# mozack/vdjer

Hardware: AMD Instinct MI355X
Metric: M paired-reads/sec (k-mer build + contig score), IgH 50bp PE (higher is better)
Workload: dtype u8/u64 (2-bit packed bases, integer counts)

## Files before the change

### vdjer_amd/csrc/vdjx_kmer.hip

```cpp
#include "vdjx_common.h"
#include "vdjx_scan.h"
#include "vdjx_part.h"

#include <algorithm>
#include <numeric>
#include <type_traits>
#include <string.h>
#include <stdlib.h>

#define HIST_THREADS 512
#define HIST_BLOCKS 512u
#define LOCAL_SLOTS 2048u
#define K3_SUB_TUPLES g_sub_tuples
__device__ u32 g_sub_tuples = 262144u;
#define NONE32 0xFFFFFFFFu
#define INST_MASK 0x7FFFFFFFu

struct RecView {
	u64 bhi, blo, nm, lq;
};

__device__ inline RecView load_rec(const u64* __restrict__ bases, const u64* __restrict__ nmask,
                                   const u64* __restrict__ lowq, size_t r) {
	RecView v;
// ... 164 lines not shown
			u32 at = incl - c;
			for (u32 gg = g; gg; gg &= gg - 1) wl[at++] = (uint16_t) ((lane << (LONG ? 8 : 6)) | (u32) (ob + __builtin_ctz(gg)));
			vdjx_wave_lds_fence();
			if (dbg == 2) { sink += wl[lane]; vdjx_wave_lds_fence(); continue; }
			for (u32 i = lane; i < total; i += 64) {
				const u32 e = wl[i];
				u64 khi, klo;
				if (LONG) vdjx_kmer_at_words(wrow + (e >> 8) * GL_ROW_LONG, k, (int) (e & 255u), khi, klo);
				else if (SYM) (void) sym_canonical(wb[e >> 6], rl, k, (int) (e & 63u), khi, klo);
				else {
					const ulonglong2 bb = wb[e >> 6];
					vdjx_kmer_at_lane(bb.x, bb.y, rl, k, (int) (e & 63u), khi, klo);
				}
				if (dbg == 3) { sink += (u32) (vdjx_bucket_mix(klo, khi) >> (64 - nb_bits)); continue; }
				atomicAdd(&hist[(u32) (vdjx_bucket_mix(klo, khi) >> (64 - nb_bits))], 1u);
			}
			vdjx_wave_lds_fence();
		}
	}
	__syncthreads();
	if (dbg) { if (sink == 0x12345u) bucket_cnt[0] = sink; return; }
	for (u32 i = threadIdx.x; i < NB; i += HIST_THREADS) if (hist[i]) atomicAdd(&bucket_cnt[i], hist[i]);
}

template <typename TUP> struct TupBucket {
	u32 shift, mask;
	__device__ inline u32 operator()(const TUP& t) const { return (u32) (vdjx_bucket_mix(t.lo, t.hi()) >> shift) & mask; }
};

#define PARTR_STAGE_BYTES 98304u
template <typename TUP, bool LONG, bool SYM = false>
__global__ __launch_bounds__(PART_THREADS) void k_part_records_g(const u64* __restrict__ bases, const u64* __restrict__ nmask,
                                                                 const u64* __restrict__ lowq, size_t R, u64 rec_base, int rl, int k,
                                                                 u32 shift, u32 nbk, size_t rpb, u32 rr0, u32* __restrict__ gcur,
                                                                 TUP* __restrict__ out) {
	extern __shared__ __attribute__((aligned(16))) uint8_t smem[];
	TUP* stage = (TUP*) smem;
	u32* desc = (u32*) (smem + PARTR_STAGE_BYTES);
	__shared__ part_round pr;
	__shared__ u32 s_n;
	constexpr u32 ROUND = PARTR_STAGE_BYTES / sizeof(TUP);
	constexpr int OB = LONG ? 8 : 6;
	const int P = rl - k + 1;
	const u32 rr_min = ROUND / (u32) P;
	u32 rr = rr0 > rr_min ? rr0 : rr_min;
	const u32 mask = nbk - 1;
	const u32 lane = threadIdx.x & 63u, wave = threadIdx.x >> 6;
	static_assert(!(LONG && SYM), "SYM is the short-read form");
	uint8_t* wv = smem + wave * (LONG ? GL_WAVE_BYTES_LONG : GL_WAVE_BYTES);
	ulonglong2* wb = (ulonglong2*) wv;
	u64* wrow = (u64*) wv;
	uint16_t* wl = (uint16_t*) (wv + (LONG ? 64u * GL_ROW_LONG * 8u : 1024u));
	const size_t r0 = (size_t) blockIdx.x * rpb;
	const size_t r1 = r0 + rpb < R ? r0 + rpb : R;
	size_t rs = r0;
	while (rs < r1) {
		const size_t re = rs + rr < r1 ? rs + rr : r1;
		if (threadIdx.x == 0) s_n = 0;
		pr.begin(nbk);
		for (size_t rb = rs; rb < re; rb += PART_THREADS) {
			const size_t r = rb + threadIdx.x;
			u64 G = 0;
			vdjx_mask3 bad{~0ull, ~0ull, ~0ull};
			if (r < re) {
				if (LONG) { bad = load_gate3(lowq, r); stage_row_long(wrow + lane * GL_ROW_LONG, bases, r); }
				else {
					const GateView v = load_gate(bases, lowq, SYM ? 2 * r : r);
// ... 7 lines not shown
				const u32 g = LONG ? vdjx_clean16(bad, ob, k, P) : (u32) (G >> ob) & 0xFFFFu;
				const u32 c = (u32) __popc(g);
				const u32 incl = (u32) vdjx_wave_scan_add((int) c);
				const u32 total = (u32) __builtin_amdgcn_readlane((int) incl, 63);
				if (!total) continue;
				u32 at = incl - c;
				for (u32 gg = g; gg; gg &= gg - 1) wl[at++] = (uint16_t) ((lane << OB) | (u32) (ob + __builtin_ctz(gg)));
				vdjx_wave_lds_fence();
				u32 dbase = 0;
				if (lane == 0) dbase = atomicAdd(&s_n, total);
				dbase = (u32) __builtin_amdgcn_readlane((int) dbase, 0);
				for (u32 i = lane; i < total; i += 64) {
					const u32 e = wl[i];
					u64 khi, klo;
					if (LONG) vdjx_kmer_at_words(wrow + (e >> 8) * GL_ROW_LONG, k, (int) (e & 255u), khi, klo);
					else if (SYM) (void) sym_canonical(wb[e >> 6], rl, k, (int) (e & 63u), khi, klo);
					else {
						const ulonglong2 bb = wb[e >> 6];
						vdjx_kmer_at_lane(bb.x, bb.y, rl, k, (int) (e & 63u), khi, klo);
					}
					const u32 b = (u32) (vdjx_bucket_mix(klo, khi) >> shift) & mask;
					pr.count(b);
					if (dbase + i < ROUND) desc[dbase + i] = ((loc0 + (e >> OB)) << (OB + 10)) | ((e & ((1u << OB) - 1u)) << 10) | b;
				}
				vdjx_wave_lds_fence();
			}
		}
		__syncthreads();
		if (s_n > ROUND) {
			rr = rr / 2 > rr_min ? rr / 2 : rr_min;
			__syncthreads();
			continue;
		}
		const u32 n = pr.reserve(nbk, gcur);
		for (u32 i = threadIdx.x; i < n; i += PART_THREADS) {
			const u32 d = desc[i];
			const size_t r = rs + (d >> (OB + 10));
			const u32 o = (d >> 10) & ((1u << OB) - 1u);
			u64 khi, klo;
			u64 inst = ((rec_base + (u64) r) << OB) | (u64) o;
			if (LONG) vdjx_kmer_at_words(bases + r * VDJX_LONG_W, k, (int) o, khi, klo);
			else if (SYM) {
				const bool flip = sym_canonical(((const ulonglong2*) bases)[2 * r], rl, k, (int) o, khi, klo);
				inst = flip ? ((rec_base + 2 * (u64) r + 1) << OB) | (u64) (rl - k - (int) o) : ((rec_base + 2 * (u64) r) << OB) | (u64) o;
			} else {
				const ulonglong2 bb = ((const ulonglong2*) bases)[r];
				vdjx_kmer_at_lane(bb.x, bb.y, rl, k, (int) o, khi, klo);
			}
			TUP::store(&stage[pr.slot(d & 1023u)], TUP::make(klo, khi, inst));
		}
		__syncthreads();
		pr.flush(stage, n, out, TupBucket<TUP>{shift, mask});
		rs = re;
	}
}

template <typename TUP>
__global__ __launch_bounds__(512) void k_seg_hist_g(const TUP* __restrict__ in, const u32* __restrict__ seg_start, u32 seg_shift, u32 slices,
                                                    u32 shift, u32 sub_bits, u32* __restrict__ fine_cnt) {
	__shared__ u32 h[PART_MAXB];
	const u32 nbk = 1u << sub_bits;
	for (u32 i = threadIdx.x; i < nbk; i += 512) h[i] = 0;
	__syncthreads();
	size_t t0, t1;
	const u32 seg = part_slice(seg_start, seg_shift, slices, t0, t1);
	for (size_t t = t0 + threadIdx.x; t < t1; t += 512) {
		const TUP x = TUP::load(&in[t]);
// ... 1607 lines not shown
	explicit PersistAlloc(vdjx_ctx* ctx) : c(ctx) {}
	template <typename T> hipError_t alloc(T** out, size_t n) {
		*out = (T*) c->shard_arena.alloc((n ? n : 1) * sizeof(T));
		return *out ? hipSuccess : hipErrorOutOfMemory;
	}
	vdjx_arena::mark_t mark() const { return c->shard_arena.mark(); }
	void release_to(vdjx_arena::mark_t m) { c->shard_arena.release_to(m); }
};

struct PoolView { const u64* bases; const u64* nmask; vdjx_qrows quals; int rl; int ob; };

template <typename TUP> struct GTuples {
	TUP* t = nullptr;
	u32* bucket_start = nullptr;
	u32 NB = 0, N = 0;
};

struct SurvivorsG {
	u64 *lo = nullptr, *hi = nullptr, *gfirst = nullptr, *ufirst = nullptr;
	u32 *gcnt = nullptr, *ucnt = nullptr;
	u32 n = 0, n_real = 0;
	u64 ndist = 0;
};

inline u32 ceil_log2_u64(u64 x) { u32 b = 0; while ((1ull << b) < x) b++; return b; }

static bool sync_debug() { static const bool on = vdjx_env_set("VDJX_SYNC_DEBUG"); return on; }
static void dbg_sync(vdjx_ctx* c, const char* what) {
	if (!sync_debug()) return;
	const hipError_t e = hipStreamSynchronize(c->stream);
	fprintf(stderr, "[vdjx] %s: %s\n", what, hipGetErrorString(e));
}

struct GatedHist { u32 HB = 0, NBH = 0, N = 0; u32* hstart = nullptr; bool sym = false; };
static bool build_sym(const vdjx_pool* pool, int k) {
	return pool->sym && pool->W == 2 && (k & 1) && pool->n_records % 2 == 0;
}
static bool sym_walk_wanted() { static const bool on = !vdjx_env_set("VDJX_NO_SYM_WALK"); return on; }
static size_t gated_bucket_default() { static const size_t v = (size_t) vdjx_env_num("VDJX_GATED_BUCKET", 3072, 1, 1ll << 32); return v; }
template <typename A>
int stage_gated_hist(vdjx_ctx* c, A& db, const vdjx_pool* pool, int k, size_t per_bucket, u64 geometry_instances, GatedHist* gh, bool sym = false) {
	hipStream_t st = c->stream;
	const size_t R = sym ? pool->n_records / 2 : pool->n_records;
	const int P = pool->rl - k + 1;
	const u64 NI = geometry_instances ? geometry_instances : (u64) R * (u64) P;
	const size_t per = per_bucket ? per_bucket : gated_bucket_default();
	const u32 hb_max = pool->W > 2 ? 14u : 15u;
	u32 HB = ceil_log2_u64((NI + per - 1) / per);
	HB = std::max(8u, std::min(hb_max, HB));
	const u32 NBH = 1u << HB;
#ifdef VDJX_ABLATE
	static const u32 hist_dbg = (u32) vdjx_env_num("VDJX_HIST_DBG", 0, 0, 4);
#else
	constexpr u32 hist_dbg = 0;
#endif
	u32 nblk = (u32) std::min<size_t>(HIST_BLOCKS, (R + 4095) / 4096);
	if (nblk == 0) nblk = 1;
	size_t rpb = (R + nblk - 1) / nblk;
	u32 *hcnt, *hstart;
	HIP_TRY(db.alloc(&hcnt, NBH));
	HIP_TRY(db.alloc(&hstart, NBH + 1));
	HIP_TRY(hipMemsetAsync(hcnt, 0, (size_t) NBH * 4, st));
	const bool lng = pool->W > 2;
	const size_t lds_hist = (size_t) NBH * 4 + (HIST_THREADS / 64) * (lng ? GL_WAVE_BYTES_LONG : GL_WAVE_BYTES);
	HIP_TRY(hipFuncSetAttribute((const void*) k_gated_hist<false>, hipFuncAttributeMaxDynamicSharedMemorySize, (int) lds_hist));
	HIP_TRY(hipFuncSetAttribute((const void*) k_gated_hist<true>, hipFuncAttributeMaxDynamicSharedMemorySize, (int) lds_hist));
	HIP_TRY(hipFuncSetAttribute((const void*) k_gated_hist<false, true>, hipFuncAttributeMaxDynamicSharedMemorySize, (int) lds_hist));
	{
		vdjx_prof_scope ps(c, "k_gated_hist");
		if (lng) hipLaunchKernelGGL(k_gated_hist<true>, dim3(nblk), dim3(HIST_THREADS), lds_hist, st, pool->d_bases, pool->d_nmask, pool->d_lowq, R, pool->rl, k, HB, rpb, hcnt, hist_dbg);
		else if (sym) hipLaunchKernelGGL((k_gated_hist<false, true>), dim3(nblk), dim3(HIST_THREADS), lds_hist, st, pool->d_bases, pool->d_nmask, pool->d_lowq, R, pool->rl, k, HB, rpb, hcnt, hist_dbg);
		else hipLaunchKernelGGL(k_gated_hist<false>, dim3(nblk), dim3(HIST_THREADS), lds_hist, st, pool->d_bases, pool->d_nmask, pool->d_lowq, R, pool->rl, k, HB, rpb, hcnt, hist_dbg);
	}
	dbg_sync(c, "k_gated_hist");
	vdjx_scan_one(st, hcnt, NBH, hstart);
	HIP_TRY(hipMemcpyAsync(c->h_pin, hstart + NBH, 4, hipMemcpyDeviceToHost, st));
	HIP_TRY(hipStreamSynchronize(st));
	HIP_TRY(hipGetLastError());
#ifdef VDJX_ABLATE
	if (hist_dbg) return VDJX_ESTATE;
#endif
	const u32 N = *(const u32*) c->h_pin;
	c->stats["gated_instances"] = sym ? 2ull * N : N;
	gh->HB = HB; gh->NBH = NBH; gh->N = N; gh->hstart = hstart; gh->sym = sym;
	return VDJX_OK;
}

template <typename TUP, typename A>
int stage_gated_cut(vdjx_ctx* c, A& db, const vdjx_pool* pool, u64 rec_base, int k, size_t per_bucket, u64 geometry_instances, const GatedHist& gh, GTuples<TUP>* out) {
	hipStream_t st = c->stream;
	const bool sym = gh.sym;
	const size_t R = sym ? pool->n_records / 2 : pool->n_records;
	const int P = pool->rl - k + 1;
	const size_t per = per_bucket ? per_bucket : gated_bucket_default();
	const u32 hb_max = pool->W > 2 ? 14u : 15u;
	const bool lng = pool->W > 2;
	const u32 HB = gh.HB, NBH = gh.NBH, N = gh.N;
	u32* hstart = gh.hstart;
	size_t rpb;
	out->N = N;
	const u64 Ng = geometry_instances ? geometry_instances : (u64) N;
	static const size_t refine = (size_t) vdjx_env_num("VDJX_REFINE_TUPLES", 4096, 1, 1ll << 32);
	u32 T = 8;
	while (T < HB && ((u64) per << T) < Ng) T++;
	u32 extra = 0;
	const size_t refine_at = per_bucket ? std::max<size_t>(per_bucket, refine / 2) : refine;
	if (T == HB && HB == hb_max && Ng / NBH > refine_at) {
		extra = 1;
		while (extra < 5 && (Ng >> extra) / NBH > refine_at) extra++;
	}
	const u32 Tt = T + extra;
	const u32 NBt = 1u << Tt;
	HIP_TRY(db.alloc(&out->t, (size_t) N + 1));
	constexpr u32 stage_tuples = PARTR_STAGE_BYTES / (u32) sizeof(TUP);
	constexpr u32 lds_partr = PARTR_STAGE_BYTES + stage_tuples * 4;
	u32 cbits = Tt, fbits = 0;
	if (Tt > 10) { cbits = extra ? Tt - 10 : 8; fbits = Tt - cbits; }
	const u32 NBc = 1u << cbits;
	u32 nblk2 = (u32) std::min<size_t>(1024, (R + 2047) / 2048);
	if (nblk2 == 0) nblk2 = 1;
	rpb = (R + nblk2 - 1) / nblk2;
	u32* gcur;
	HIP_TRY(db.alloc(&gcur, NBc));
	TUP* l1 = out->t;
	if (fbits) HIP_TRY(db.alloc(&l1, (size_t) N + 1));
	{
		vdjx_prof_scope ps(c, "k_part_records");
		const u64 NIl = (u64) R * (u64) P;
		u64 rr = N ? (u64) stage_tuples * 3 / 4 * NIl / ((u64) N * (u64) P) : 1u << 16;
		rr = std::max<u64>(PART_THREADS, std::min<u64>(rr / PART_THREADS * PART_THREADS, lng ? 1u << 14 : 1u << 16));
		auto* part_records = lng ? k_part_records_g<TUP, true> : sym ? k_part_records_g<TUP, false, true> : k_part_records_g<TUP, false>;
		HIP_TRY(part_launch(st, part_records, nblk2, lds_partr, hstart, NBc, HB - cbits, gcur, l1, pool->d_bases, pool->d_nmask, pool->d_lowq, R, rec_base,
		                    pool->rl, k, 64 - cbits, NBc, rpb, (u32) rr));
	}
	dbg_sync(c, "k_part_records");
	u32* tstart;
	HIP_TRY(db.alloc(&tstart, NBt + 1));
	out->NB = NBt;
	out->bucket_start = tstart;
	constexpr u32 slices = PART_SLICES;
	if (extra) {
		u32* fine_cnt;
		HIP_TRY(db.alloc(&fine_cnt, NBt));
		HIP_TRY(hipMemsetAsync(fine_cnt, 0, (size_t) NBt * 4, st));
		vdjx_prof_scope ps(c, "k_seg_hist");
		hipLaunchKernelGGL(k_seg_hist_g<TUP>, dim3(NBc * slices), dim3(512), 0, st, l1, hstart, HB - cbits, slices, 64 - Tt, fbits, fine_cnt);
		vdjx_scan_one(st, fine_cnt, NBt, tstart);
	} else {
		hipLaunchKernelGGL(k_pick_u32, dim3((NBt + 1 + 255) / 256), dim3(256), 0, st, hstart, 1u << (HB - Tt), NBt + 1, tstart);
	}
	if (fbits) {
		u32* gcur2;
		HIP_TRY(db.alloc(&gcur2, NBt));
		vdjx_prof_scope ps(c, "k_part_tuples");
		HIP_TRY(part_launch(st, k_part<TUP, TupBucket<TUP>, part_segs>, NBc * slices, PART_LDS_BYTES, tstart, NBt, 0u, gcur2, out->t,
		                    l1, part_segs{hstart, HB - cbits, slices, fbits}, TupBucket<TUP>{64 - Tt, (1u << fbits) - 1u}));
	}
	return VDJX_OK;
}

template <typename TUP, typename A>
int stage_gated_partition(vdjx_ctx* c, A& db, const vdjx_pool* pool, u64 rec_base, int k, size_t per_bucket, u64 geometry_instances, GTuples<TUP>* out, bool sym = false) {
	GatedHist gh;
	int rc = stage_gated_hist(c, db, pool, k, per_bucket, geometry_instances, &gh, sym);
	if (rc) return rc;
	return stage_gated_cut<TUP>(c, db, pool, rec_base, k, per_bucket, geometry_instances, gh, out);
}

static int set_sub_tuples(vdjx_ctx* c) {
	static const u32 sub = (u32) vdjx_env_num("VDJX_SUB_TUPLES", 262144, 1, 0xFFFFFFFFll);
	if (c->sub_tuples_set != sub) {
		HIP_TRY(hipMemcpyToSymbolAsync(HIP_SYMBOL(g_sub_tuples), &sub, 4, 0, hipMemcpyHostToDevice, c->stream));
		c->sub_tuples_set = sub;
	}
	return VDJX_OK;
}
template <typename TUP, typename A>
int bucket_order(vdjx_ctx* c, A& db, const GTuples<TUP>& t, u32** order) {
	*order = nullptr;
	if (t.NB < 1024) return VDJX_OK;
	HIP_TRY(db.alloc(order, t.NB));
	hipLaunchKernelGGL(k_bucket_order, dim3(1), dim3(1024), 0, c->stream, t.bucket_start, t.NB, *order);
	return VDJX_OK;
}

template <typename TUP, typename A>
int stage_gated_reduce(vdjx_ctx* c, A& db, const GTuples<TUP>& t, const PoolView& pv, u64 rec_base, int k, int mf, int mq, SurvivorsG* sv, bool sym = false) {
	hipStream_t st = c->stream;
	int rc = set_sub_tuples(c);
// ... 150 lines not shown
		u32 x = f.mul;
		for (int i = 0; i < 5; i++) x *= 2u - f.mul * x;
		f.inv = x & f.bmask;
		f.ns = ns;
	}
	const u32 nsp = (f.bmask + 1u) << 4;
	static const bool force_wide = vdjx_env_num("VDJX_RC_WIDE", 0, 0, 1) != 0;
	static const u32 cap_shift = (u32) vdjx_env_num("VDJX_RC_MAX_SHIFT", 12, 8, 12);
	const bool narrow = R < (1ull << (32 - pool->ob)) && !force_wide;
	static const u32 max_ranges = (u32) vdjx_env_num("VDJX_RC_MAX_RANGES", PART_MAXB, 2, PART_MAXB);
	const u32 max_shift = std::max(8u, std::min(narrow ? 11u : 10u, cap_shift));
	u32 range_shift = 8;
	while (range_shift < max_shift && (nsp >> range_shift) > max_ranges) range_shift++;
	const u32 n_ranges = std::max(1u, nsp >> range_shift);
	u32 l2bits = 0;
	while (((n_ranges + (1u << l2bits) - 1) >> l2bits) > max_ranges) l2bits++;
	if (l2bits) l2bits = std::min(10u, std::max(l2bits, (ceil_log2_u64(n_ranges) + 1u) / 2u));
	const u32 n_coarse = (n_ranges + (1u << l2bits) - 1) >> l2bits;
	const u32 n_ranges_p = n_coarse << l2bits;
	constexpr size_t walk_blocks = 7168;
	const size_t Rw = sym_walk ? R / 2 : R;
	u32 nblk = (u32) std::min<size_t>(walk_blocks, (Rw + WALK_THREADS * 8 - 1) / (WALK_THREADS * 8));
	constexpr u32 walk_resident = 1536;
	if (nblk > walk_resident && nblk < walk_blocks) nblk = nblk / walk_resident * walk_resident;
	if (nblk < walk_resident) nblk = (u32) std::min<size_t>(walk_resident, (Rw + WALK_THREADS - 1) / WALK_THREADS);
	if (nblk == 0) nblk = 1;
	const size_t nwaves = (size_t) nblk * (WALK_THREADS / 64);
	const size_t NI = R * (size_t) P;
	u32 blk_items = 4096;
	while (blk_items > 256 && nwaves * blk_items > NI / 2 + 65536) blk_items >>= 1;
	const u64 raw_cap = (u64) NI + (u64) NI / (blk_items / 64) + nwaves * (u64) blk_items + blk_items;
	u64 *raw, *items;
	unsigned long long *g_cursor, *n_inst;
	u32 *range_cnt, *range_start, *g_err, *gcur;
	const vdjx_arena::mark_t tmp_mark = db.mark();
	HIP_TRY(db.alloc(&raw, (size_t) raw_cap));
	HIP_TRY(db.alloc(&g_cursor, 4 + ((size_t) n_ranges_p + 1) / 2));
	n_inst = g_cursor + 1;
	g_err = (u32*) (g_cursor + 2);
	range_cnt = (u32*) (g_cursor + 4);
	HIP_TRY(db.alloc(&range_start, n_ranges_p + 1));
	HIP_TRY(hipMemsetAsync(g_cursor, 0, 32 + (size_t) n_ranges_p * 4, st));
	if (sym_walk) {
		vdjx_prof_scope ps(c, "k_chain_order");
		hipLaunchKernelGGL(k_partner_check, gs, bs, 0, st, partner, linw, ns, g_err + 3);
	}
	const bool lng = pool->W > 2;
	if (lng && R >= (1ull << 27)) { vdjx_set_error("more than 2^27 records of long reads on one GPU: not supported by the recount items"); return VDJX_ELIMIT; }
	const size_t lds_walk = (((size_t) n_ranges_p + 1) & ~(size_t) 1) * 4 + (lng ? (size_t) WALK_THREADS * GL_ROW_LONG * 8 : 0);
	if ((size_t) n_ranges_p * 4 > 64 * 1024) { vdjx_set_error("too many survivor ranges for the walk histogram"); return VDJX_ELIMIT; }
	HIP_TRY(hipFuncSetAttribute((const void*) k_walk_items<false>, hipFuncAttributeMaxDynamicSharedMemorySize, (int) lds_walk));
	HIP_TRY(hipFuncSetAttribute((const void*) k_walk_items<true>, hipFuncAttributeMaxDynamicSharedMemorySize, (int) lds_walk));
	HIP_TRY(hipFuncSetAttribute((const void*) k_walk_items<false, true>, hipFuncAttributeMaxDynamicSharedMemorySize, (int) lds_walk));
#ifdef VDJX_ABLATE
	static const u32 walk_dbg = (u32) vdjx_env_num("VDJX_WALK_DBG", 0, 0, 63);
#else
	constexpr u32 walk_dbg = 0;
#endif
	if (R && walk_dbg != 0u) {
		u64* raw2;
		unsigned long long* cur2;
		u32* cnt2;
		HIP_TRY(db.alloc(&raw2, (size_t) raw_cap));
		HIP_TRY(db.alloc(&cur2, 8));
		HIP_TRY(db.alloc(&cnt2, n_ranges_p));
		HIP_TRY(hipMemsetAsync(cur2, 0, 64, st));
		HIP_TRY(hipMemsetAsync(cnt2, 0, (size_t) n_ranges_p * 4, st));
		vdjx_prof_scope ps(c, "k_walk_dbg");
		if (lng) hipLaunchKernelGGL(k_walk_items<true>, dim3(nblk), dim3(WALK_THREADS), lds_walk, st, pool->d_bases, pool->d_nmask, R, pool->rl, pool->ob, k, tb, succ, linw, f, range_shift,
		                            n_ranges_p, raw2, raw_cap, blk_items, cur2, cnt2, g_err, walk_dbg, (const u32*) nullptr);
		else hipLaunchKernelGGL(k_walk_items<false>, dim3(nblk), dim3(WALK_THREADS), lds_walk, st, pool->d_bases, pool->d_nmask, R, pool->rl, pool->ob, k, tb, succ, linw, f, range_shift,
		                        n_ranges_p, raw2, raw_cap, blk_items, cur2, cnt2, g_err, walk_dbg, (const u32*) nullptr);
		HIP_TRY(hipMemsetAsync(g_err, 0, 4, st));
		if (walk_dbg & 32u) {
			unsigned long long hs[8];
			HIP_TRY(hipMemcpyAsync(hs, cur2, 64, hipMemcpyDeviceToHost, st));
			HIP_TRY(hipStreamSynchronize(st));
			const char* nm[] = {"", "rows", "rounds", "filter", "lookup", "chain", "item_trips"};
			for (int i = 1; i < 7; i++) c->stats[std::string("walk_dbg_") + nm[i]] = hs[i];
		}
	}
	if (R) {
		vdjx_prof_scope ps(c, "k_walk_items");
		if (lng) hipLaunchKernelGGL(k_walk_items<true>, dim3(nblk), dim3(WALK_THREADS), lds_walk, st, pool->d_bases, pool->d_nmask, R, pool->rl, pool->ob, k, tb, succ, linw, f, range_shift,
		                            n_ranges_p, raw, raw_cap, blk_items, g_cursor, range_cnt, g_err, 0u, (const u32*) nullptr);
		else if (sym_walk) hipLaunchKernelGGL((k_walk_items<false, true>), dim3(nblk), dim3(WALK_THREADS), lds_walk, st, pool->d_bases, pool->d_nmask, R / 2, pool->rl, pool->ob, k, tb, succ, linw, f, range_shift,
		                                      n_ranges_p, raw, raw_cap, blk_items, g_cursor, range_cnt, g_err, 0u, (const u32*) partner);
		else hipLaunchKernelGGL(k_walk_items<false>, dim3(nblk), dim3(WALK_THREADS), lds_walk, st, pool->d_bases, pool->d_nmask, R, pool->rl, pool->ob, k, tb, succ, linw, f, range_shift,
		                        n_ranges_p, raw, raw_cap, blk_items, g_cursor, range_cnt, g_err, 0u, (const u32*) nullptr);
	}
	dbg_sync(c, "k_walk_items");
	vdjx_scan_one(st, range_cnt, n_ranges_p, range_start);
	size_t items_cap = NI + 1;
	if (!defer) {
		u32* hp = (u32*) c->h_pin;
		HIP_TRY(hipMemcpyAsync(hp, range_start + n_ranges_p, 4, hipMemcpyDeviceToHost, st));
		HIP_TRY(hipStreamSynchronize(st));
		HIP_TRY(hipGetLastError());
		items_cap = (size_t) hp[0] + 1;
	}
	HIP_TRY(db.alloc(&items, items_cap));
	HIP_TRY(db.alloc(&gcur, n_ranges_p));
	{
		vdjx_prof_scope ps(c, "k_part_items");
		u32 npb = (u32) std::min<size_t>(1024, (NI / 4 + 65535) / 65536);
		if (npb == 0) npb = 1;
		const auto k_part_items = k_part<u64, ItemRange, part_share, true>;
		if (!l2bits) {
			HIP_TRY(part_launch(st, k_part_items, npb, PART_LDS_BYTES, range_start, n_ranges_p, 0u, gcur, items, raw, part_share{g_cursor, n_ranges_p},
			                    ItemRange{f, range_shift, ~0u}));
		} else {
			u64* l1;
			u32* gcur1;
			HIP_TRY(db.alloc(&l1, items_cap));
			HIP_TRY(db.alloc(&gcur1, n_coarse));
			HIP_TRY(part_launch(st, k_part_items, npb, PART_LDS_BYTES, range_start, n_coarse, l2bits, gcur1, l1, raw, part_share{g_cursor, n_coarse},
			                    ItemRange{f, range_shift + l2bits, ~0u}));
			const u32 sl2 = std::max(8u, std::min(64u, 2048u / n_coarse));
			HIP_TRY(part_launch(st, k_part<u64, ItemRange, part_segs>, n_coarse * sl2, PART_LDS_BYTES, range_start, n_ranges_p, 0u, gcur, items,
			                    l1, part_segs{range_start, l2bits, sl2, l2bits}, ItemRange{f, range_shift, (1u << l2bits) - 1u}));
		}
	}
	dbg_sync(c, "k_part_items");
	{
		vdjx_prof_scope ps(c, "k_recount");
#define RC_LAUNCH(SB, IT) hipLaunchKernelGGL((k_recount<SB, IT>), dim3(n_ranges), dim3(RC_THREADS), 0, st, items, range_start, f, ns, rec_base, pool->ob, fbw, ro.ucnt, ro.ufirst, ro.in_first, n_inst)
		if (narrow) {
			switch (range_shift) {
				case 8: RC_LAUNCH(256, u32); break;
				case 9: RC_LAUNCH(512, u32); break;
				case 10: RC_LAUNCH(1024, u32); break;
				default: RC_LAUNCH(2048, u32); break;
			}
		} else {
			switch (range_shift) {
				case 8: RC_LAUNCH(256, u64); break;
				case 9: RC_LAUNCH(512, u64); break;
				default: RC_LAUNCH(1024, u64); break;
			}
		}
#undef RC_LAUNCH
	}
	dbg_sync(c, "k_recount");
	if (derive_edges) {
		hipLaunchKernelGGL(k_count_unseen, dim3((ns + 255) / 256), dim3(256), 0, st, ro.ufirst, ns, g_err + 1);
		HIP_TRY(hipMemsetAsync(ro.edge_first, 0xFF, (size_t) ns * 32, st));
		hipLaunchKernelGGL(k_edges_from_in, dim3((ns * 4 + 255) / 256), dim3(256), 0, st, tb, ns, k, ro.in_first, ro.in_from, ro.edge_first, ro.edge_to);
	}
	if (defer && !sync_debug()) {
		defer->g_err = g_err; defer->n_items = range_start + n_ranges_p; defer->n_inst = n_inst; defer->ns = ns;
		return VDJX_OK;
	}
	if (defer) defer->g_err = nullptr;
// ... 759 lines not shown
	if (!vdjx_ctx_alive(g->ctx)) { vdjx_set_error("vdjx_graph_export_end: the graph's context is gone"); return VDJX_ESTATE; }
	HIP_TRY(hipSetDevice(g->device));
	HIP_TRY(hipStreamSynchronize(g->ctx->copy_stream));
	return VDJX_OK;
}

extern "C" void vdjx_graph_free(vdjx_graph* g) {
	if (!g) return;
	if (g->d_block) {
		(void) hipSetDevice(g->device);
		if (vdjx_ctx_alive(g->ctx)) {
			(void) hipStreamSynchronize(g->ctx->copy_stream);
			g->ctx->blocks.release(g->d_block, g->block_cap);
		}
		else vdjx_block_cache::discard(g->d_block);
	}
	delete g;
}

struct PartTestKey {
	u32 shift, mask;
	__device__ inline u32 operator()(u64 x) const { return ((u32) (x >> 40) >> shift) & mask; }
	__device__ inline u32 operator()(const Tup16& t) const { return (*this)(t.lo); }
};

template <typename T, bool PAIRED>
static int part_test(vdjx_ctx* c, const void* host_in, size_t n, const std::vector<u32>& cnt, int levels, u32 fine_bits, u32 slices, u32 workgroups,
                     u32* host_starts, void* host_out) {
	hipStream_t st = c->stream;
	vdjx_work db(c);
	const u32 nb = (u32) cnt.size(), coarse = nb >> fine_bits;
	const unsigned long long n_raw = n;
	T *d_in, *d_l1, *d_out;
	u32 *d_cnt, *d_starts, *gcur, *gcur1;
	unsigned long long* d_n;
	HIP_TRY(db.alloc(&d_in, n + 1));
	HIP_TRY(db.alloc(&d_l1, n + 1));
	HIP_TRY(db.alloc(&d_out, n + 1));
	HIP_TRY(db.alloc(&d_cnt, nb));
	HIP_TRY(db.alloc(&d_starts, nb + 1));
	HIP_TRY(db.alloc(&gcur, nb));
	HIP_TRY(db.alloc(&gcur1, coarse));
	HIP_TRY(db.alloc(&d_n, 1));
	if (n) HIP_TRY(hipMemcpyAsync(d_in, host_in, n * sizeof(T), hipMemcpyHostToDevice, st));
	HIP_TRY(hipMemcpyAsync(d_cnt, cnt.data(), (size_t) nb * 4, hipMemcpyHostToDevice, st));
	HIP_TRY(hipMemcpyAsync(d_n, &n_raw, 8, hipMemcpyHostToDevice, st));
	vdjx_scan_one(st, (const u32*) d_cnt, nb, d_starts);
	const auto level1 = k_part<T, PartTestKey, part_share, PAIRED>;
	if (levels == 1) {
		HIP_TRY(part_launch(st, level1, workgroups, PART_LDS_BYTES, d_starts, nb, 0u, gcur, d_out, d_in, part_share{d_n, nb}, PartTestKey{0u, ~0u}));
	} else {
		HIP_TRY(part_launch(st, level1, workgroups, PART_LDS_BYTES, d_starts, coarse, fine_bits, gcur1, d_l1, d_in, part_share{d_n, coarse},
		                    PartTestKey{fine_bits, ~0u}));
		HIP_TRY(part_launch(st, k_part<T, PartTestKey, part_segs>, coarse * slices, PART_LDS_BYTES, d_starts, nb, 0u, gcur, d_out, d_l1,
		                    part_segs{d_starts, fine_bits, slices, fine_bits}, PartTestKey{0u, (1u << fine_bits) - 1u}));
	}
	const size_t kept = std::accumulate(cnt.begin(), cnt.end(), (size_t) 0);
	HIP_TRY(hipMemcpyAsync(host_starts, d_starts, ((size_t) nb + 1) * 4, hipMemcpyDeviceToHost, st));
	if (kept) HIP_TRY(hipMemcpyAsync(host_out, d_out, kept * sizeof(T), hipMemcpyDeviceToHost, st));
	HIP_TRY(hipStreamSynchronize(st));
	HIP_TRY(hipGetLastError());
	return VDJX_OK;
}

extern "C" int vdjx_part_u64(vdjx_ctx* c, const void* host_in, size_t n, int elem_bytes, uint32_t nb, int levels, uint32_t fine_bits, uint32_t slices,
                             uint32_t workgroups, uint32_t* host_starts, void* host_out) {
	const auto refuse = [](const char* what) { vdjx_set_error("vdjx_part_u64: %s", what); return VDJX_EINVAL; };
	if (!c || !host_starts || (n && (!host_in || !host_out)) || n >= (1ull << 31)) return refuse("bad argument");
	if (elem_bytes != 8 && elem_bytes != 16) return refuse("elements of 8 or 16 bytes");
	if (levels != 1 && levels != 2) return refuse("one level or two");
	if (slices == 0 || slices > 1024 || workgroups == 0 || workgroups > 65536) return refuse("1 .. 1024 slices, 1 .. 65536 workgroups");
	if (levels == 1) fine_bits = 0;
	if (fine_bits > 10) return refuse("at most 10 fine bits");
	if (nb == 0 || (nb >> fine_bits) > PART_MAXB || (nb >> fine_bits) << fine_bits != nb) return refuse("nb is at most 1024, or coarse << fine_bits with coarse <= 1024");
	std::vector<u32> cnt(nb, 0u);
	const u64* w = (const u64*) host_in;
	for (size_t i = 0; i < n; i++) {
		const u64 x = w[i * (size_t) (elem_bytes / 8)];
		if (elem_bytes == 8 && x == PART_HOLE) continue;
		if ((x >> 40) >= nb) return refuse("the bucket of an element is not below nb");
		cnt[(size_t) (x >> 40)]++;
	}
	HIP_TRY(hipSetDevice(c->device));
	vdjx_clear_errors();
	if (elem_bytes == 8) return part_test<u64, true>(c, host_in, n, cnt, levels, fine_bits, slices, workgroups, host_starts, host_out);
	return part_test<Tup16, false>(c, host_in, n, cnt, levels, fine_bits, slices, workgroups, host_starts, host_out);
}
```

### vdjer_amd/csrc/vdjx_part.h

```cpp
#pragma once

#include "vdjx_common.h"

#include <type_traits>

#define PART_THREADS 1024
#define PART_LDS_BYTES 131072
#define PART_MAXB 1024
#define PART_SLICES 8u
#define PART_NONE 0xFFFFFFFFu
#define PART_HOLE 0xFFFFFFFFFFFFFFFFull

namespace {

__device__ inline void part_scan(const u32* cnt, u32* base, u32* tmp, u32 n) {
	const u32 t = threadIdx.x, lane = t & 63, wv = t >> 6;
	const u32 a = 2 * t < n ? cnt[2 * t] : 0, b = 2 * t + 1 < n ? cnt[2 * t + 1] : 0;
	const u32 incl = (u32) vdjx_wave_scan_add((int) (a + b));
	if (lane == 63) tmp[wv] = incl;
	__syncthreads();
	if (wv == 0) {
		const u32 w = lane < PART_THREADS / 64 ? tmp[lane] : 0;
		const u32 wi = (u32) vdjx_wave_scan_add((int) w);
		if (lane < PART_THREADS / 64) tmp[lane] = wi - w;
		if (lane == 63) tmp[PART_THREADS / 64] = wi;
	}
	__syncthreads();
	const u32 excl = tmp[wv] + incl - (a + b);
	if (2 * t < n) base[2 * t] = excl;
	if (2 * t + 1 < n) base[2 * t + 1] = excl + a;
	if (t == 0) base[n] = tmp[PART_THREADS / 64];
	__syncthreads();
}

template <typename T> __device__ inline T part_load(const T* p) { return T::load(p); }
template <typename T> __device__ inline void part_store(T* p, const T& x) { T::store(p, x); }
__device__ inline u64 part_load(const u64* p) { return *p; }
__device__ inline void part_store(u64* p, const u64& x) { *p = x; }

struct part_round {
	u32 cnt[PART_MAXB], base[PART_MAXB + 1], cur[PART_MAXB], gbase[PART_MAXB], tmp[PART_THREADS];

	__device__ inline void begin(u32 nbk) {
		for (u32 i = threadIdx.x; i < nbk; i += PART_THREADS) cnt[i] = 0;
		__syncthreads();
	}
	__device__ inline void count(u32 b) { atomicAdd(&cnt[b], 1u); }
	__device__ inline u32 reserve(u32 nbk, u32* __restrict__ gcur) {
		part_scan(cnt, base, tmp, nbk);
		for (u32 i = threadIdx.x; i < nbk; i += PART_THREADS) {
			cur[i] = base[i];
			gbase[i] = cnt[i] ? atomicAdd(&gcur[i], cnt[i]) : 0u;
		}
		__syncthreads();
		return base[nbk];
	}
	__device__ inline u32 slot(u32 b) { return atomicAdd(&cur[b], 1u); }
	template <typename T, typename Key> __device__ inline void flush(const T* stage, u32 n, T* __restrict__ out, const Key& key) {
		for (u32 i = threadIdx.x; i < n; i += PART_THREADS) {
			const T x = part_load(&stage[i]);
			const u32 b = key(x);
			part_store(&out[gbase[b] + (i - base[b])], x);
		}
		__syncthreads();
	}
};

__device__ inline u32 part_slice(const u32* __restrict__ seg_start, u32 seg_shift, u32 slices, size_t& t0, size_t& t1) {
	const u32 seg = blockIdx.x / slices, sl = blockIdx.x % slices;
	const size_t s0 = seg_start[(size_t) seg << seg_shift], s1 = seg_start[((size_t) seg + 1) << seg_shift];
	const size_t per = (s1 - s0 + slices - 1) / slices;
	t0 = s0 + (size_t) sl * per;
	t1 = t0 + per < s1 ? t0 + per : s1;
	return seg;
}

struct part_share {
	const unsigned long long* n;
	u32 nbk;
	__device__ inline size_t span(u32 round, size_t& t0, size_t& t1, u32& buckets) const {
		const size_t N = (size_t) *n;
		const size_t per = ((N + gridDim.x - 1) / gridDim.x + round - 1) / round * round;
		t0 = (size_t) blockIdx.x * per;
		t1 = t0 + per < N ? t0 + per : N;
		buckets = nbk;
		return 0;
	}
};
struct part_segs {
	const u32* seg_start;
	u32 seg_shift, slices, sub_bits;
	__device__ inline size_t span(u32, size_t& t0, size_t& t1, u32& buckets) const {
		buckets = 1u << sub_bits;
		return (size_t) part_slice(seg_start, seg_shift, slices, t0, t1) << sub_bits;
	}
};

template <typename T, typename Key, typename Range, bool PAIRED = false>
__global__ __launch_bounds__(PART_THREADS) void k_part(const T* __restrict__ in, Range range, Key key, u32* __restrict__ gcur, T* __restrict__ out) {
	extern __shared__ __attribute__((aligned(16))) uint8_t part_smem[];
	T* stage = (T*) part_smem;
	__shared__ part_round pr;
	constexpr u32 PER = PART_LDS_BYTES / sizeof(T) / PART_THREADS;
	constexpr u32 ROUND = PER * PART_THREADS;
	static_assert(!PAIRED || (std::is_same<T, u64>::value && PER % 2 == 0), "the paired loads are for 8-byte elements");
	size_t t0, t1;
	u32 nbk;
	u32* gc = gcur + range.span(ROUND, t0, t1, nbk);
	for (size_t ts = t0; ts < t1; ts += ROUND) {
		const size_t te = ts + ROUND < t1 ? ts + ROUND : t1;
		pr.begin(nbk);
		T r_x[PER];
		u32 r_b[PER];
		if constexpr (PAIRED) {
#pragma unroll
			for (u32 j = 0; j < PER; j += 2) {
				const size_t t = ts + ((size_t) (j / 2) * PART_THREADS + threadIdx.x) * 2;
				r_x[j] = PART_HOLE; r_x[j + 1] = PART_HOLE;
				if (t + 1 < te) { const ulonglong2 v = *(const ulonglong2*) &in[t]; r_x[j] = v.x; r_x[j + 1] = v.y; }
				else if (t < te) r_x[j] = in[t];
			}
#pragma unroll
			for (u32 j = 0; j < PER; j++) {
				r_b[j] = PART_NONE;
				if (r_x[j] != PART_HOLE) { r_b[j] = key(r_x[j]); pr.count(r_b[j]); }
			}
		} else {
#pragma unroll
			for (u32 j = 0; j < PER; j++) {
				const size_t t = ts + (size_t) j * PART_THREADS + threadIdx.x;
				r_b[j] = PART_NONE;
				if (t < te) { r_x[j] = part_load(&in[t]); r_b[j] = key(r_x[j]); }
			}
#pragma unroll
			for (u32 j = 0; j < PER; j++) if (r_b[j] != PART_NONE) pr.count(r_b[j]);
		}
		__syncthreads();
		const u32 n = pr.reserve(nbk, gc);
#pragma unroll
		for (u32 j = 0; j < PER; j++) if (r_b[j] != PART_NONE) part_store(&stage[pr.slot(r_b[j])], r_x[j]);
		__syncthreads();
		pr.flush(stage, n, out, key);
	}
}

__global__ void k_init_cursors(const u32* __restrict__ bucket_start, u32 n, u32 sh, u32* __restrict__ cur) {
	u32 i = blockIdx.x * blockDim.x + threadIdx.x;
	if (i < n) cur[i] = bucket_start[(size_t) i << sh];
}

template <typename... P, typename O, typename... Args>
inline hipError_t part_launch(hipStream_t st, void (*kernel)(P...), u32 grid, u32 lds, const u32* bucket_start, u32 ncur, u32 sh, u32* gcur, O* out,
                              Args... args) {
	const hipError_t e = hipFuncSetAttribute((const void*) kernel, hipFuncAttributeMaxDynamicSharedMemorySize, (int) lds);
	if (e != hipSuccess) return e;
	hipLaunchKernelGGL(k_init_cursors, dim3((ncur + 255) / 256), dim3(256), 0, st, bucket_start, ncur, sh, gcur);
	hipLaunchKernelGGL(kernel, dim3(grid), dim3(PART_THREADS), lds, st, args..., gcur, out);
	return hipSuccess;
}

}
```

Baseline: 909.9.

## Drop cursor-init kernels, deal segment rounds dynamically, prefetch next partition round

The separate k_init_cursors launch is removed. Cursors now start at zero, come from memsets folded into existing allocations, and have the bucket start added at reserve time. Segmented partition passes no longer split each segment into static slices. Blocks draw round tickets from a per-segment atomic counter, which balances uneven segments. The partition kernel also software-prefetches the next round's input into registers while the current round is staged and flushed, at the cost of more register pressure and an extra atomic per round.

```diff
diff --git a/vdjer_amd/csrc/vdjx_kmer.hip b/vdjer_amd/csrc/vdjx_kmer.hip
--- a/vdjer_amd/csrc/vdjx_kmer.hip
+++ b/vdjer_amd/csrc/vdjx_kmer.hip
@@ -220,7 +220,7 @@
 template <typename TUP, bool LONG, bool SYM = false>
 __global__ __launch_bounds__(PART_THREADS) void k_part_records_g(const u64* __restrict__ bases, const u64* __restrict__ nmask,
                                                                  const u64* __restrict__ lowq, size_t R, u64 rec_base, int rl, int k,
-                                                                 u32 shift, u32 nbk, size_t rpb, u32 rr0, u32* __restrict__ gcur,
+                                                                 u32 shift, u32 nbk, size_t rpb, u32 rr0, part_cursors pc,
                                                                  TUP* __restrict__ out) {
 	extern __shared__ __attribute__((aligned(16))) uint8_t smem[];
 	TUP* stage = (TUP*) smem;
@@ -294,7 +294,7 @@
 			__syncthreads();
 			continue;
 		}
-		const u32 n = pr.reserve(nbk, gcur);
+		const u32 n = pr.reserve(nbk, pc);
 		for (u32 i = threadIdx.x; i < n; i += PART_THREADS) {
 			const u32 d = desc[i];
 			const size_t r = rs + (d >> (OB + 10));
@@ -1968,7 +1968,7 @@
 	fprintf(stderr, "[vdjx] %s: %s\n", what, hipGetErrorString(e));
 }
 
-struct GatedHist { u32 HB = 0, NBH = 0, N = 0; u32* hstart = nullptr; bool sym = false; };
+struct GatedHist { u32 HB = 0, NBH = 0, N = 0; u32* hstart = nullptr; bool sym = false; u32* zero = nullptr; };
 static bool build_sym(const vdjx_pool* pool, int k) {
 	return pool->sym && pool->W == 2 && (k & 1) && pool->n_records % 2 == 0;
 }
@@ -1994,9 +1994,10 @@
 	if (nblk == 0) nblk = 1;
 	size_t rpb = (R + nblk - 1) / nblk;
 	u32 *hcnt, *hstart;
-	HIP_TRY(db.alloc(&hcnt, NBH));
+	const size_t n_zero = (size_t) NBH + 2 * PART_MAXB;
+	HIP_TRY(db.alloc(&hcnt, NBH + n_zero));
 	HIP_TRY(db.alloc(&hstart, NBH + 1));
-	HIP_TRY(hipMemsetAsync(hcnt, 0, (size_t) NBH * 4, st));
+	HIP_TRY(hipMemsetAsync(hcnt, 0, ((size_t) NBH + n_zero) * 4, st));
 	const bool lng = pool->W > 2;
 	const size_t lds_hist = (size_t) NBH * 4 + (HIST_THREADS / 64) * (lng ? GL_WAVE_BYTES_LONG : GL_WAVE_BYTES);
 	HIP_TRY(hipFuncSetAttribute((const void*) k_gated_hist<false>, hipFuncAttributeMaxDynamicSharedMemorySize, (int) lds_hist));
@@ -2018,12 +2019,12 @@
 #endif
 	const u32 N = *(const u32*) c->h_pin;
 	c->stats["gated_instances"] = sym ? 2ull * N : N;
-	gh->HB = HB; gh->NBH = NBH; gh->N = N; gh->hstart = hstart; gh->sym = sym;
+	gh->HB = HB; gh->NBH = NBH; gh->N = N; gh->hstart = hstart; gh->sym = sym; gh->zero = hcnt + NBH;
 	return VDJX_OK;
 }
 
 template <typename TUP, typename A>
-int stage_gated_cut(vdjx_ctx* c, A& db, const vdjx_pool* pool, u64 rec_base, int k, size_t per_bucket, u64 geometry_instances, const GatedHist& gh, GTuples<TUP>* out) {
+int stage_gated_cut(vdjx_ctx* c, A& db, const vdjx_pool* pool, u64 rec_base, int k, size_t per_bucket, u64 geometry_instances, GatedHist& gh, GTuples<TUP>* out) {
 	hipStream_t st = c->stream;
 	const bool sym = gh.sym;
 	const size_t R = sym ? pool->n_records / 2 : pool->n_records;
@@ -2056,8 +2057,14 @@
 	u32 nblk2 = (u32) std::min<size_t>(1024, (R + 2047) / 2048);
 	if (nblk2 == 0) nblk2 = 1;
 	rpb = (R + nblk2 - 1) / nblk2;
-	u32* gcur;
-	HIP_TRY(db.alloc(&gcur, NBc));
+	const size_t n_zero = (size_t) NBH + 2 * PART_MAXB;
+	u32* zero = gh.zero;
+	gh.zero = nullptr;
+	if (!zero) {
+		HIP_TRY(db.alloc(&zero, n_zero));
+		HIP_TRY(hipMemsetAsync(zero, 0, n_zero * 4, st));
+	}
+	u32 *gcur = zero, *ticket2 = zero + PART_MAXB, *gcur2 = zero + 2 * PART_MAXB;
 	TUP* l1 = out->t;
 	if (fbits) HIP_TRY(db.alloc(&l1, (size_t) N + 1));
 	{
@@ -2066,7 +2073,7 @@
 		u64 rr = N ? (u64) stage_tuples * 3 / 4 * NIl / ((u64) N * (u64) P) : 1u << 16;
 		rr = std::max<u64>(PART_THREADS, std::min<u64>(rr / PART_THREADS * PART_THREADS, lng ? 1u << 14 : 1u << 16));
 		auto* part_records = lng ? k_part_records_g<TUP, true> : sym ? k_part_records_g<TUP, false, true> : k_part_records_g<TUP, false>;
-		HIP_TRY(part_launch(st, part_records, nblk2, lds_partr, hstart, NBc, HB - cbits, gcur, l1, pool->d_bases, pool->d_nmask, pool->d_lowq, R, rec_base,
+		HIP_TRY(part_launch(st, part_records, nblk2, lds_partr, part_cursors{hstart, HB - cbits, gcur}, l1, pool->d_bases, pool->d_nmask, pool->d_lowq, R, rec_base,
 		                    pool->rl, k, 64 - cbits, NBc, rpb, (u32) rr));
 	}
 	dbg_sync(c, "k_part_records");
@@ -2077,8 +2084,9 @@
 	constexpr u32 slices = PART_SLICES;
 	if (extra) {
 		u32* fine_cnt;
-		HIP_TRY(db.alloc(&fine_cnt, NBt));
-		HIP_TRY(hipMemsetAsync(fine_cnt, 0, (size_t) NBt * 4, st));
+		HIP_TRY(db.alloc(&fine_cnt, 2 * (size_t) NBt));
+		HIP_TRY(hipMemsetAsync(fine_cnt, 0, 2 * (size_t) NBt * 4, st));
+		gcur2 = fine_cnt + NBt;
 		vdjx_prof_scope ps(c, "k_seg_hist");
 		hipLaunchKernelGGL(k_seg_hist_g<TUP>, dim3(NBc * slices), dim3(512), 0, st, l1, hstart, HB - cbits, slices, 64 - Tt, fbits, fine_cnt);
 		vdjx_scan_one(st, fine_cnt, NBt, tstart);
@@ -2086,11 +2094,9 @@
 		hipLaunchKernelGGL(k_pick_u32, dim3((NBt + 1 + 255) / 256), dim3(256), 0, st, hstart, 1u << (HB - Tt), NBt + 1, tstart);
 	}
 	if (fbits) {
-		u32* gcur2;
-		HIP_TRY(db.alloc(&gcur2, NBt));
 		vdjx_prof_scope ps(c, "k_part_tuples");
-		HIP_TRY(part_launch(st, k_part<TUP, TupBucket<TUP>, part_segs>, NBc * slices, PART_LDS_BYTES, tstart, NBt, 0u, gcur2, out->t,
-		                    l1, part_segs{hstart, HB - cbits, slices, fbits}, TupBucket<TUP>{64 - Tt, (1u << fbits) - 1u}));
+		HIP_TRY(part_launch(st, k_part<TUP, TupBucket<TUP>, part_segs>, NBc * slices, PART_LDS_BYTES, part_cursors{tstart, 0u, gcur2}, out->t,
+		                    l1, part_segs{hstart, HB - cbits, slices, fbits, ticket2}, TupBucket<TUP>{64 - Tt, (1u << fbits) - 1u}));
 	}
 	return VDJX_OK;
 }
@@ -2307,15 +2313,19 @@
 	const u64 raw_cap = (u64) NI + (u64) NI / (blk_items / 64) + nwaves * (u64) blk_items + blk_items;
 	u64 *raw, *items;
 	unsigned long long *g_cursor, *n_inst;
-	u32 *range_cnt, *range_start, *g_err, *gcur;
+	u32 *range_cnt, *range_start, *g_err, *gcur, *gcur1, *ticket2;
 	const vdjx_arena::mark_t tmp_mark = db.mark();
 	HIP_TRY(db.alloc(&raw, (size_t) raw_cap));
-	HIP_TRY(db.alloc(&g_cursor, 4 + ((size_t) n_ranges_p + 1) / 2));
+	const size_t n_clear = 2 * (size_t) n_ranges_p + 2 * (size_t) n_coarse;
+	HIP_TRY(db.alloc(&g_cursor, 4 + (n_clear + 1) / 2));
 	n_inst = g_cursor + 1;
 	g_err = (u32*) (g_cursor + 2);
 	range_cnt = (u32*) (g_cursor + 4);
+	gcur = range_cnt + n_ranges_p;
+	gcur1 = gcur + n_ranges_p;
+	ticket2 = gcur1 + n_coarse;
 	HIP_TRY(db.alloc(&range_start, n_ranges_p + 1));
-	HIP_TRY(hipMemsetAsync(g_cursor, 0, 32 + (size_t) n_ranges_p * 4, st));
+	HIP_TRY(hipMemsetAsync(g_cursor, 0, 32 + n_clear * 4, st));
 	if (sym_walk) {
 		vdjx_prof_scope ps(c, "k_chain_order");
 		hipLaunchKernelGGL(k_partner_check, gs, bs, 0, st, partner, linw, ns, g_err + 3);
@@ -2375,25 +2385,22 @@
 		items_cap = (size_t) hp[0] + 1;
 	}
 	HIP_TRY(db.alloc(&items, items_cap));
-	HIP_TRY(db.alloc(&gcur, n_ranges_p));
 	{
 		vdjx_prof_scope ps(c, "k_part_items");
 		u32 npb = (u32) std::min<size_t>(1024, (NI / 4 + 65535) / 65536);
 		if (npb == 0) npb = 1;
 		const auto k_part_items = k_part<u64, ItemRange, part_share, true>;
 		if (!l2bits) {
-			HIP_TRY(part_launch(st, k_part_items, npb, PART_LDS_BYTES, range_start, n_ranges_p, 0u, gcur, items, raw, part_share{g_cursor, n_ranges_p},
+			HIP_TRY(part_launch(st, k_part_items, npb, PART_LDS_BYTES, part_cursors{range_start, 0u, gcur}, items, raw, part_share{g_cursor, n_ranges_p},
 			                    ItemRange{f, range_shift, ~0u}));
 		} else {
 			u64* l1;
-			u32* gcur1;
 			HIP_TRY(db.alloc(&l1, items_cap));
-			HIP_TRY(db.alloc(&gcur1, n_coarse));
-			HIP_TRY(part_launch(st, k_part_items, npb, PART_LDS_BYTES, range_start, n_coarse, l2bits, gcur1, l1, raw, part_share{g_cursor, n_coarse},
+			HIP_TRY(part_launch(st, k_part_items, npb, PART_LDS_BYTES, part_cursors{range_start, l2bits, gcur1}, l1, raw, part_share{g_cursor, n_coarse},
 			                    ItemRange{f, range_shift + l2bits, ~0u}));
 			const u32 sl2 = std::max(8u, std::min(64u, 2048u / n_coarse));
-			HIP_TRY(part_launch(st, k_part<u64, ItemRange, part_segs>, n_coarse * sl2, PART_LDS_BYTES, range_start, n_ranges_p, 0u, gcur, items,
-			                    l1, part_segs{range_start, l2bits, sl2, l2bits}, ItemRange{f, range_shift, (1u << l2bits) - 1u}));
+			HIP_TRY(part_launch(st, k_part<u64, ItemRange, part_segs>, n_coarse * sl2, PART_LDS_BYTES, part_cursors{range_start, 0u, gcur}, items,
+			                    l1, part_segs{range_start, l2bits, sl2, l2bits, ticket2}, ItemRange{f, range_shift, (1u << l2bits) - 1u}));
 		}
 	}
 	dbg_sync(c, "k_part_items");
@@ -3219,15 +3226,17 @@
 	const u32 nb = (u32) cnt.size(), coarse = nb >> fine_bits;
 	const unsigned long long n_raw = n;
 	T *d_in, *d_l1, *d_out;
-	u32 *d_cnt, *d_starts, *gcur, *gcur1;
+	u32 *d_cnt, *d_starts, *gcur, *gcur1, *ticket2;
 	unsigned long long* d_n;
 	HIP_TRY(db.alloc(&d_in, n + 1));
 	HIP_TRY(db.alloc(&d_l1, n + 1));
 	HIP_TRY(db.alloc(&d_out, n + 1));
 	HIP_TRY(db.alloc(&d_cnt, nb));
 	HIP_TRY(db.alloc(&d_starts, nb + 1));
-	HIP_TRY(db.alloc(&gcur, nb));
-	HIP_TRY(db.alloc(&gcur1, coarse));
+	HIP_TRY(db.alloc(&gcur, (size_t) nb + 2 * (size_t) coarse));
+	gcur1 = gcur + nb;
+	ticket2 = gcur1 + coarse;
+	HIP_TRY(hipMemsetAsync(gcur, 0, ((size_t) nb + 2 * (size_t) coarse) * 4, st));
 	HIP_TRY(db.alloc(&d_n, 1));
 	if (n) HIP_TRY(hipMemcpyAsync(d_in, host_in, n * sizeof(T), hipMemcpyHostToDevice, st));
 	HIP_TRY(hipMemcpyAsync(d_cnt, cnt.data(), (size_t) nb * 4, hipMemcpyHostToDevice, st));
@@ -3235,12 +3244,12 @@
 	vdjx_scan_one(st, (const u32*) d_cnt, nb, d_starts);
 	const auto level1 = k_part<T, PartTestKey, part_share, PAIRED>;
 	if (levels == 1) {
-		HIP_TRY(part_launch(st, level1, workgroups, PART_LDS_BYTES, d_starts, nb, 0u, gcur, d_out, d_in, part_share{d_n, nb}, PartTestKey{0u, ~0u}));
+		HIP_TRY(part_launch(st, level1, workgroups, PART_LDS_BYTES, part_cursors{d_starts, 0u, gcur}, d_out, d_in, part_share{d_n, nb}, PartTestKey{0u, ~0u}));
 	} else {
-		HIP_TRY(part_launch(st, level1, workgroups, PART_LDS_BYTES, d_starts, coarse, fine_bits, gcur1, d_l1, d_in, part_share{d_n, coarse},
+		HIP_TRY(part_launch(st, level1, workgroups, PART_LDS_BYTES, part_cursors{d_starts, fine_bits, gcur1}, d_l1, d_in, part_share{d_n, coarse},
 		                    PartTestKey{fine_bits, ~0u}));
-		HIP_TRY(part_launch(st, k_part<T, PartTestKey, part_segs>, coarse * slices, PART_LDS_BYTES, d_starts, nb, 0u, gcur, d_out, d_l1,
-		                    part_segs{d_starts, fine_bits, slices, fine_bits}, PartTestKey{0u, (1u << fine_bits) - 1u}));
+		HIP_TRY(part_launch(st, k_part<T, PartTestKey, part_segs>, coarse * slices, PART_LDS_BYTES, part_cursors{d_starts, 0u, gcur}, d_out, d_l1,
+		                    part_segs{d_starts, fine_bits, slices, fine_bits, ticket2}, PartTestKey{0u, (1u << fine_bits) - 1u}));
 	}
 	const size_t kept = std::accumulate(cnt.begin(), cnt.end(), (size_t) 0);
 	HIP_TRY(hipMemcpyAsync(host_starts, d_starts, ((size_t) nb + 1) * 4, hipMemcpyDeviceToHost, st));
diff --git a/vdjer_amd/csrc/vdjx_part.h b/vdjer_amd/csrc/vdjx_part.h
--- a/vdjer_amd/csrc/vdjx_part.h
+++ b/vdjer_amd/csrc/vdjx_part.h
@@ -38,19 +38,30 @@
 __device__ inline u64 part_load(const u64* p) { return *p; }
 __device__ inline void part_store(u64* p, const u64& x) { *p = x; }
 
+struct part_cursors {
+	const u32* start;
+	u32 sh;
+	u32* cur;
+};
+
 struct part_round {
 	u32 cnt[PART_MAXB], base[PART_MAXB + 1], cur[PART_MAXB], gbase[PART_MAXB], tmp[PART_THREADS];
+	u32 next;
 
 	__device__ inline void begin(u32 nbk) {
 		for (u32 i = threadIdx.x; i < nbk; i += PART_THREADS) cnt[i] = 0;
 		__syncthreads();
 	}
 	__device__ inline void count(u32 b) { atomicAdd(&cnt[b], 1u); }
-	__device__ inline u32 reserve(u32 nbk, u32* __restrict__ gcur) {
+	__device__ inline void draw(u32* __restrict__ deal) {
+		if (threadIdx.x == PART_THREADS - 1) next = atomicAdd(deal, 1u);
+	}
+	__device__ inline u32 reserve(u32 nbk, const part_cursors& pc, u32* __restrict__ deal = nullptr) {
 		part_scan(cnt, base, tmp, nbk);
+		if (deal) draw(deal);
 		for (u32 i = threadIdx.x; i < nbk; i += PART_THREADS) {
 			cur[i] = base[i];
-			gbase[i] = cnt[i] ? atomicAdd(&gcur[i], cnt[i]) : 0u;
+			gbase[i] = cnt[i] ? pc.start[(size_t) i << pc.sh] + atomicAdd(&pc.cur[i], cnt[i]) : 0u;
 		}
 		__syncthreads();
 		return base[nbk];
@@ -76,86 +87,110 @@
 }
 
 struct part_share {
+	static constexpr bool DEALT = false;
 	const unsigned long long* n;
 	u32 nbk;
-	__device__ inline size_t span(u32 round, size_t& t0, size_t& t1, u32& buckets) const {
+	__device__ inline size_t span(u32 round, size_t& t0, size_t& t1, u32& buckets, u32*& deal) const {
 		const size_t N = (size_t) *n;
 		const size_t per = ((N + gridDim.x - 1) / gridDim.x + round - 1) / round * round;
 		t0 = (size_t) blockIdx.x * per;
 		t1 = t0 + per < N ? t0 + per : N;
 		buckets = nbk;
+		deal = nullptr;
 		return 0;
 	}
 };
 struct part_segs {
+	static constexpr bool DEALT = true;
 	const u32* seg_start;
 	u32 seg_shift, slices, sub_bits;
-	__device__ inline size_t span(u32, size_t& t0, size_t& t1, u32& buckets) const {
+	u32* ticket;
+	__device__ inline size_t span(u32, size_t& t0, size_t& t1, u32& buckets, u32*& deal) const {
+		const u32 seg = blockIdx.x / slices;
+		t0 = seg_start[(size_t) seg << seg_shift];
+		t1 = seg_start[((size_t) seg + 1) << seg_shift];
 		buckets = 1u << sub_bits;
-		return (size_t) part_slice(seg_start, seg_shift, slices, t0, t1) << sub_bits;
+		deal = ticket + seg;
+		return (size_t) seg << sub_bits;
 	}
 };
 
 template <typename T, typename Key, typename Range, bool PAIRED = false>
-__global__ __launch_bounds__(PART_THREADS) void k_part(const T* __restrict__ in, Range range, Key key, u32* __restrict__ gcur, T* __restrict__ out) {
+__global__ __launch_bounds__(PART_THREADS) void k_part(const T* __restrict__ in, Range range, Key key, part_cursors pc, T* __restrict__ out) {
 	extern __shared__ __attribute__((aligned(16))) uint8_t part_smem[];
 	T* stage = (T*) part_smem;
 	__shared__ part_round pr;
 	constexpr u32 PER = PART_LDS_BYTES / sizeof(T) / PART_THREADS;
 	constexpr u32 ROUND = PER * PART_THREADS;
 	static_assert(!PAIRED || (std::is_same<T, u64>::value && PER % 2 == 0), "the paired loads are for 8-byte elements");
+	static_assert(!PAIRED || !Range::DEALT, "a dealt range starts anywhere");
 	size_t t0, t1;
 	u32 nbk;
-	u32* gc = gcur + range.span(ROUND, t0, t1, nbk);
-	for (size_t ts = t0; ts < t1; ts += ROUND) {
+	u32* deal;
+	const size_t c0 = range.span(ROUND, t0, t1, nbk, deal);
+	pc.start += c0 << pc.sh;
+	pc.cur += c0;
+	const auto load = [&](size_t ts, T (&x)[PER]) {
 		const size_t te = ts + ROUND < t1 ? ts + ROUND : t1;
-		pr.begin(nbk);
-		T r_x[PER];
-		u32 r_b[PER];
 		if constexpr (PAIRED) {
 #pragma unroll
 			for (u32 j = 0; j < PER; j += 2) {
 				const size_t t = ts + ((size_t) (j / 2) * PART_THREADS + threadIdx.x) * 2;
-				r_x[j] = PART_HOLE; r_x[j + 1] = PART_HOLE;
-				if (t + 1 < te) { const ulonglong2 v = *(const ulonglong2*) &in[t]; r_x[j] = v.x; r_x[j + 1] = v.y; }
-				else if (t < te) r_x[j] = in[t];
-			}
-#pragma unroll
-			for (u32 j = 0; j < PER; j++) {
-				r_b[j] = PART_NONE;
-				if (r_x[j] != PART_HOLE) { r_b[j] = key(r_x[j]); pr.count(r_b[j]); }
+				x[j] = PART_HOLE; x[j + 1] = PART_HOLE;
+				if (t + 1 < te) { const ulonglong2 v = *(const ulonglong2*) &in[t]; x[j] = v.x; x[j + 1] = v.y; }
+				else if (t < te) x[j] = in[t];
 			}
 		} else {
 #pragma unroll
 			for (u32 j = 0; j < PER; j++) {
 				const size_t t = ts + (size_t) j * PART_THREADS + threadIdx.x;
-				r_b[j] = PART_NONE;
-				if (t < te) { r_x[j] = part_load(&in[t]); r_b[j] = key(r_x[j]); }
+				x[j] = T{};
+				if (t < te) x[j] = part_load(&in[t]);
 			}
+		}
+	};
+	size_t ts = t0;
+	if constexpr (Range::DEALT) {
+		pr.draw(deal);
+		__syncthreads();
+		ts = t0 + (size_t) pr.next * ROUND;
+	}
+	T r_x[PER];
+	load(ts, r_x);
+	while (ts < t1) {
+		const size_t te = ts + ROUND < t1 ? ts + ROUND : t1;
+		pr.begin(nbk);
+		u32 r_b[PER];
 #pragma unroll
-			for (u32 j = 0; j < PER; j++) if (r_b[j] != PART_NONE) pr.count(r_b[j]);
+		for (u32 j = 0; j < PER; j++) {
+			bool there;
+			if constexpr (PAIRED) there = r_x[j] != PART_HOLE;
+			else there = ts + (size_t) j * PART_THREADS + threadIdx.x < te;
+			const u32 b = key(r_x[j]);
+			r_b[j] = there ? b : PART_NONE;
 		}
+#pragma unroll
+		for (u32 j = 0; j < PER; j++) if (r_b[j] != PART_NONE) pr.count(r_b[j]);
 		__syncthreads();
-		const u32 n = pr.reserve(nbk, gc);
+		const u32 n = pr.reserve(nbk, pc, deal);
+		const size_t tn = Range::DEALT ? t0 + (size_t) pr.next * ROUND : ts + ROUND;
+		T r_n[PER];
+		load(tn, r_n);
 #pragma unroll
 		for (u32 j = 0; j < PER; j++) if (r_b[j] != PART_NONE) part_store(&stage[pr.slot(r_b[j])], r_x[j]);
 		__syncthreads();
 		pr.flush(stage, n, out, key);
+#pragma unroll
+		for (u32 j = 0; j < PER; j++) r_x[j] = r_n[j];
+		ts = tn;
 	}
 }
 
-__global__ void k_init_cursors(const u32* __restrict__ bucket_start, u32 n, u32 sh, u32* __restrict__ cur) {
-	u32 i = blockIdx.x * blockDim.x + threadIdx.x;
-	if (i < n) cur[i] = bucket_start[(size_t) i << sh];
-}
-
 template <typename... P, typename O, typename... Args>
-inline hipError_t part_launch(hipStream_t st, void (*kernel)(P...), u32 grid, u32 lds, const u32* bucket_start, u32 ncur, u32 sh, u32* gcur, O* out,
-                              Args... args) {
+inline hipError_t part_launch(hipStream_t st, void (*kernel)(P...), u32 grid, u32 lds, part_cursors pc, O* out, Args... args) {
 	const hipError_t e = hipFuncSetAttribute((const void*) kernel, hipFuncAttributeMaxDynamicSharedMemorySize, (int) lds);
 	if (e != hipSuccess) return e;
-	hipLaunchKernelGGL(k_init_cursors, dim3((ncur + 255) / 256), dim3(256), 0, st, bucket_start, ncur, sh, gcur);
-	hipLaunchKernelGGL(kernel, dim3(grid), dim3(PART_THREADS), lds, st, args..., gcur, out);
+	hipLaunchKernelGGL(kernel, dim3(grid), dim3(PART_THREADS), lds, st, args..., pc, out);
 	return hipSuccess;
 }
 
```

Result: no change. 904.6 (-0.6%).
